# sadit/Jchemo.jl

Measured on AMD Instinct MI355X. Metric: latent-variables/sec (plskern n=1e6 p=500 q=10 nlv=25), higher is better.
Workload: dtype f64

## Files before the change

### jchemo.jl_amd/csrc/deflate.hip

```cpp
#include <stdlib.h>

#include <algorithm>

#include "jch_internal.h"

typedef double v4f64 __attribute__((ext_vector_type(4)));
#define XT_LD 65
#define YT_LD 17

template <bool APPLY, bool STORE>
__global__ __launch_bounds__(256) void k_deflate_xty(double *__restrict__ Xr, int64_t n, int p, int ldr,
                                                      const double *__restrict__ Yr, int qpad, int q, int yg0,
                                                      const double *__restrict__ d, const double *__restrict__ tcol,
                                                      const double *__restrict__ zpc, double *__restrict__ Kpart,
                                                      int kp_rows)
{
    __shared__ double xt[64 * XT_LD];
    __shared__ double yt[64 * YT_LD];
    __shared__ double tl[64], dl[64];
    const int tid = threadIdx.x, lane = tid & 63, wv = tid >> 6;
    const int j0 = blockIdx.y * 64;
    const int yg = yg0 + blockIdx.z;
    const int64_t nchunks = (n + 63) / 64;
    const int jcol = j0 + lane;
// ... 537 lines not shown
    int64_t c = blockIdx.x;
    int cur = 0;
    if (c < nchunks) { fetch(c); stage(0); }
    __syncthreads();
    for (; c < nchunks; c += gridDim.x) {
        const int64_t i0 = c * RB;
        v2f64 x[STEPS][NS];
#pragma unroll
        for (int st = 0; st < STEPS; ++st)
#pragma unroll
            for (int u = 0; u < NS; ++u) x[st][u] = xn[st][u];
        const bool more = c + gridDim.x < nchunks;
        if (more) fetch(c + gridDim.x);
#pragma unroll
        for (int st = 0; st < STEPS; ++st) {
            const int lr = 4 * st + g;
            const int64_t r = i0 + lr;
#pragma unroll
            for (int k = 0; k < MP; ++k) {
                if (k < npend) {
                    const double t = tl[cur][k][lr];
#pragma unroll
                    for (int u = 0; u < NS; ++u) {
                        x[st][u].x -= t * pk[k][u][0];
                        x[st][u].y -= t * pk[k][u][1];
                    }
                }
            }
            const double b = bt[cur][lr][c16];
#pragma unroll
            for (int u = 0; u < NS; ++u) {
                acc[u][0] = __builtin_amdgcn_mfma_f64_16x16x4f64(x[st][u].x, b, acc[u][0], 0, 0, 0);
                acc[u][1] = __builtin_amdgcn_mfma_f64_16x16x4f64(x[st][u].y, b, acc[u][1], 0, 0, 0);
            }
            if (flush && r < n) {
                double *wp = Xr + (size_t)r * (size_t)ldr;
#pragma unroll
                for (int u = 0; u < NS; ++u)
                    if (in[u]) __builtin_nontemporal_store(x[st][u], reinterpret_cast<v2f64 *>(wp + coff[u]));
            }
        }
        if (more) stage(cur ^ 1);
        __syncthreads();
        cur ^= 1;
    }
    if (Kpart) {
        double *kp = Kpart + (size_t)blockIdx.x * kp_rows * 16;
#pragma unroll
        for (int u = 0; u < NS; ++u)
#pragma unroll
            for (int h = 0; h < 2; ++h)
#pragma unroll
                for (int reg = 0; reg < 4; ++reg) {
                    const int j = 32 * (wv + 4 * u) + 2 * (4 * reg + g) + h;
                    if (j < kp_rows) kp[(size_t)j * 16 + c16] = acc[u][h][reg];
                }
    }
}

template <int NS, int STEPS, int MP>
static int32_t launch_kpass_mfma_lazy_t(jch_ctx *ctx, double *Xr, int64_t n, int p, int ldr, double *Yr, int q, const double *d,
                                        const double *pend_p, int npend, const double *tpend, int64_t tstride, const double *cvec,
                                        bool flush, double *Knext)
{
    constexpr int RB = 4 * STEPS;
    if (npend > MP) return jch_fail(ctx, JCH_EINVAL, "internal: lazy MFMA pass: %d pending corrections, at most %d", npend, MP);
    const int64_t nchunks = (n + RB - 1) / RB;
    const int nb = (int)std::max<int64_t>(std::min<int64_t>(nchunks, (int64_t)ctx->cus), 1);
    const int kp_rows = ldr;
    JCH_TRY(jch_reserve(ctx, ctx->kpart, sizeof(double) * (size_t)nb * kp_rows * 16));
    double *Kpart = (double *)ctx->kpart.ptr;
    (void)jch_ev(ctx);
    hipLaunchKernelGGL((k_kpass_mfma_lazy<NS, STEPS, MP>), dim3(nb), dim3(256), 0, ctx->stream, Xr, n, ldr, Yr, q, d, pend_p,
                       jch_nipals_lazy_pitch(ldr), npend, tpend, tstride, cvec, flush ? 1 : 0, Knext ? Kpart : nullptr, kp_rows);
    (void)jch_ev(ctx);
    if (Knext) {
        hipLaunchKernelGGL(k_reduce_kpart3, dim3((p * 16 + 63) / 64), dim3(1024), 0, ctx->stream, Kpart, nb, kp_rows * 16, p * 16, Knext);
        JCH_TRY(jch_allreduce_f64(ctx, Knext, (size_t)p * 16));
    }
    JCH_HIP(ctx, hipGetLastError());
    return JCH_OK;
}

static bool lazy_stream_shape(int ldr, int q) { return q >= 1 && q <= 4 && ldr <= 2048 && !(ldr > 1024 && q > 2); }

static int32_t launch_kpass_tile_lazy(jch_ctx *ctx, double *Xr, int64_t n, int p, int ldr, double *Yr, int qpad, int q, const double *d,
                                      const double *pend_p, int npend, const double *tpend, int64_t tstride, const double *cvec, bool flush,
                                      double *Knext)
{
    const int ptiles = (ldr + 63) / 64, kp_rows = ptiles * 64;
    const int64_t nchunks = (n + 63) / 64;
    int nbx = (ctx->cus * 3 + ptiles - 1) / ptiles;
    if (nbx > nchunks) nbx = (int)(nchunks > 0 ? nchunks : 1);
    double *Kpart = nullptr;
    if (Knext) {
        JCH_TRY(jch_reserve(ctx, ctx->kpart, sizeof(double) * (size_t)nbx * kp_rows * qpad));
        Kpart = (double *)ctx->kpart.ptr;
    }
    (void)jch_ev(ctx);
    hipLaunchKernelGGL(k_kpass_tile_lazy, dim3(nbx, ptiles, 1), dim3(256), 0, ctx->stream, Xr, n, ldr, Yr, qpad, q, d, pend_p,
                       jch_nipals_lazy_pitch(ldr), npend, tpend, tstride, cvec, flush ? 1 : 0, Kpart, kp_rows);
    (void)jch_ev(ctx);
    const int nby = (int)std::min<int64_t>((n * qpad + 255) / 256, (int64_t)ctx->cus * 8);
    hipLaunchKernelGGL(k_deflate_y, dim3(nby > 0 ? nby : 1), dim3(256), 0, ctx->stream, Yr, n, qpad, q, tpend + (size_t)(npend - 1) * tstride, cvec);
    if (Knext) {
        hipLaunchKernelGGL(k_reduce_kpart2, dim3((p * qpad + 255) / 256), dim3(256), 0, ctx->stream, Kpart, nbx, kp_rows, p, qpad, Knext);
        JCH_TRY(jch_allreduce_f64(ctx, Knext, (size_t)p * qpad));
    }
    JCH_HIP(ctx, hipGetLastError());
    return JCH_OK;
}

int32_t jch_launch_kpass_lazy(jch_ctx *ctx, double *Xr, int64_t n, int p, int ldr, double *Yr, int qpad, int q, const double *d,
                              const double *pend_p, int npend, int npend_max, const double *tpend, int64_t tstride,
                              const double *cvec, bool flush, double *Knext)
{
    if (npend < 1 || npend > npend_max || npend_max > jch_nipals_lazy_capacity(ldr, q))
        return jch_fail(ctx, JCH_EINVAL, "internal: lazy NIPALS pass: bad pending count");
    if (!lazy_stream_shape(ldr, q)) {
        if (qpad == 16 && ldr <= 1024) {
#define JCH_KM(NS, STEPS, MP) return launch_kpass_mfma_lazy_t<NS, STEPS, MP>(ctx, Xr, n, p, ldr, Yr, q, d, pend_p, npend, tpend, tstride, cvec, flush, Knext)
            if (ldr <= 128) JCH_KM(1, 4, 6);
            if (ldr <= 256) JCH_KM(2, 4, 6);
            if (ldr <= 512) JCH_KM(4, 4, 6);
            JCH_KM(8, 2, 3);
#undef JCH_KM
        }
        return launch_kpass_tile_lazy(ctx, Xr, n, p, ldr, Yr, qpad, q, d, pend_p, npend, tpend, tstride, cvec, flush, Knext);
    }
#define JCH_KL(KC, R) do { \
        if (q == 1) return launch_kpass_lazy_t<KC, R, 1>(ctx, Xr, n, p, ldr, Yr, qpad, d, pend_p, npend, npend_max, tpend, tstride, cvec, flush, Knext); \
        if (q == 2) return launch_kpass_lazy_t<KC, R, 2>(ctx, Xr, n, p, ldr, Yr, qpad, d, pend_p, npend, npend_max, tpend, tstride, cvec, flush, Knext); \
        return launch_kpass_lazy_t<KC, R, 4>(ctx, Xr, n, p, ldr, Yr, qpad, d, pend_p, npend, npend_max, tpend, tstride, cvec, flush, Knext); } while (0)
    if (ldr <= 128) JCH_KL(1, 4);
    if (ldr <= 256) JCH_KL(2, 4);
    if (ldr <= 512) JCH_KL(4, 2);
    if (ldr <= 1024) JCH_KL(8, 1);
    if (q == 1) return launch_kpass_lazy_t<16, 2, 1>(ctx, Xr, n, p, ldr, Yr, qpad, d, pend_p, npend, npend_max, tpend, tstride, cvec, flush, Knext);
    return launch_kpass_lazy_t<16, 1, 2>(ctx, Xr, n, p, ldr, Yr, qpad, d, pend_p, npend, npend_max, tpend, tstride, cvec, flush, Knext);
#undef JCH_KL
}

int32_t jch_launch_deflate(jch_ctx *ctx, double *Xr, int64_t n, int p, int ldr, double *Yr, int qpad, int q,
                           const double *d, const double *tcol, const double *zpc, double *Knext)
{
    if (q <= 4) {
#define JCH_DS(KC, R) do { \
        if (q == 1) return launch_deflate_stream<KC, R, 1>(ctx, Xr, n, p, ldr, Yr, qpad, d, tcol, zpc, Knext); \
        if (q == 2) return launch_deflate_stream<KC, R, 2>(ctx, Xr, n, p, ldr, Yr, qpad, d, tcol, zpc, Knext); \
        return launch_deflate_stream<KC, R, 4>(ctx, Xr, n, p, ldr, Yr, qpad, d, tcol, zpc, Knext); } while (0)
        if (ldr <= 128) JCH_DS(1, 4);
        if (ldr <= 256) JCH_DS(2, 4);
        if (ldr <= 512) JCH_DS(4, 2);
        if (ldr <= 1024) JCH_DS(8, 1);
        if (ldr <= 2048) {
            if (q == 1) return launch_deflate_stream<16, 2, 1>(ctx, Xr, n, p, ldr, Yr, qpad, d, tcol, zpc, Knext);
            if (q == 2) return launch_deflate_stream<16, 1, 2>(ctx, Xr, n, p, ldr, Yr, qpad, d, tcol, zpc, Knext);
        }
#undef JCH_DS
    }
    const int ptiles = (ldr + 63) / 64, kp_rows = ptiles * 64, ygroups = qpad / 16;
    const int64_t nchunks = (n + 63) / 64;
    int nbx = (ctx->cus * 3 + ptiles - 1) / ptiles;
    if (nbx > nchunks) nbx = (int)(nchunks > 0 ? nchunks : 1);
    double *Kpart = nullptr;
    if (Knext) {
        JCH_TRY(jch_reserve(ctx, ctx->kpart, sizeof(double) * (size_t)nbx * kp_rows * qpad));
        Kpart = (double *)ctx->kpart.ptr;
    }
    (void)jch_ev(ctx);
    hipLaunchKernelGGL((k_deflate_xty<true, true>), dim3(nbx, ptiles, 1), dim3(256), 0, ctx->stream, Xr, n, p, ldr, Yr, qpad,
                       q, 0, d, tcol, zpc, Kpart, kp_rows);
    (void)jch_ev(ctx);
    const int nby = (int)std::min<int64_t>((n * qpad + 255) / 256, (int64_t)ctx->cus * 8);
    hipLaunchKernelGGL(k_deflate_y, dim3(nby > 0 ? nby : 1), dim3(256), 0, ctx->stream, Yr, n, qpad, q, tcol, zpc + ldr);
    if (Knext && ygroups > 1)
        hipLaunchKernelGGL((k_deflate_xty<false, false>), dim3(nbx, ptiles, ygroups - 1), dim3(256), 0, ctx->stream, Xr, n, p,
                           ldr, Yr, qpad, q, 1, d, tcol, zpc, Kpart, kp_rows);
    if (Knext) {
        hipLaunchKernelGGL(k_reduce_kpart2, dim3((p * qpad + 255) / 256), dim3(256), 0, ctx->stream, Kpart, nbx, kp_rows, p,
                           qpad, Knext);
        JCH_TRY(jch_allreduce_f64(ctx, Knext, (size_t)p * qpad));
    }
    JCH_HIP(ctx, hipGetLastError());
    return JCH_OK;
}
```

### jchemo.jl_amd/csrc/fit.hip

```cpp
#include <stdlib.h>
#include <time.h>

#include <algorithm>
#include <condition_variable>
#include <mutex>
#include <thread>

#include "jch_internal.h"

__global__ __launch_bounds__(256) void k_fill_const(double *__restrict__ v, int m, double c)
{
    const int j = blockIdx.x * 256 + threadIdx.x;
    if (j < m) v[j] = c;
}

__global__ __launch_bounds__(256) void k_nan_zero_weight_rows(double *__restrict__ T, int64_t n, int nlv, const double *__restrict__ d)
{
    const int64_t i = (int64_t)blockIdx.x * 256 + threadIdx.x;
    if (i < n && d[i] == 0.0)
        for (int a = 0; a < nlv; ++a) T[(size_t)i + (size_t)a * (size_t)n] = __builtin_nan("");
}

__global__ __launch_bounds__(256) void k_widen_bf16(const unsigned short *__restrict__ src, int64_t ld, int64_t n, int64_t cols, double *__restrict__ dst)
{
// ... 164 lines not shown
    double tl_h2d = tl0, tl_enq = tl0, tl_sync = tl0;

    const xcopy_key xkey{io.X, (int64_t)n, (int64_t)io.ldx, p, host ? 1 : 0};
    const bool reuse_x = (d.reserved & JCH_REUSE_XCOPY) && allow_raw && ctx->xcopy_valid && ctx->xcopy == xkey && d.dtype == JCH_F64 &&
                         q + 1 <= 12 && ldr <= 512 && !jch_knob_set("JCH_NO_REUSE_XCOPY");
    if (!reuse_x) ctx->xcopy_valid = false;
    double *Xc = (double *)io.X, *Yc = (double *)io.Y;
    const double *wdev = io.weights;
    int64_t ldxc = io.ldx, ldyc = io.ldy;
    if (host) {
        JCH_TRY(jch_reserve_xstage(ctx, sizeof(double) * (size_t)n * p, reuse_x));
        JCH_TRY(jch_reserve(ctx, ctx->ystage, sizeof(double) * (size_t)n * q));
        Xc = (double *)ctx->xstage.ptr; Yc = (double *)ctx->ystage.ptr; ldxc = n; ldyc = n;
        if (!reuse_x) JCH_TRY(jch_copy2d(ctx, Xc, n, (const double *)io.X, io.ldx, n, p, hipMemcpyHostToDevice));
        JCH_TRY(jch_copy2d(ctx, Yc, n, (const double *)io.Y, io.ldy, n, q, hipMemcpyHostToDevice));
        if (io.weights) {
            JCH_TRY(jch_reserve(ctx, ctx->wstage, sizeof(double) * (size_t)n));
            JCH_HIP(ctx, hipMemcpyAsync(ctx->wstage.ptr, io.weights, sizeof(double) * (size_t)n, hipMemcpyHostToDevice, ctx->stream));
            wdev = (const double *)ctx->wstage.ptr;
        }
    }
    if (host && host_timing) { (void)hipStreamSynchronize(ctx->stream); tl_h2d = now_ms(); }
    const int nlv_cap = (int)std::min<int64_t>(d.nlv, p);
    if (d.dtype == JCH_F64) {
        JCH_TRY(jch_reserve_xr(ctx, sizeof(double) * (size_t)n * ldr, reuse_x));
        JCH_TRY(jch_reserve(ctx, ctx->yr, sizeof(double) * (size_t)n * qpad));
    }
    double *Xr = (double *)ctx->xr.ptr, *Yr = (double *)ctx->yr.ptr;
    double *dn = nullptr;
    if (!host && io.weights_norm) dn = io.weights_norm;
    else { JCH_TRY(jch_reserve(ctx, ctx->dnorm, sizeof(double) * (size_t)n)); dn = (double *)ctx->dnorm.ptr; }
    double *Tdev = nullptr;
    if (!host && io.T) Tdev = io.T;
    else { JCH_TRY(jch_reserve(ctx, ctx->tbuf, sizeof(double) * (size_t)n * nlv_cap)); Tdev = (double *)ctx->tbuf.ptr; }

    t_column_copier tcopy(ctx, (host && d.dtype == JCH_F64 && !(algo == ALGO_WOLD && (d.reserved & JCH_WOLD_REF_ZERO_WEIGHT_NAN))) ? io.T : nullptr, Tdev, n, nlv_cap);
    const size_t small_bytes = 256 * 21 + sizeof(double) * 16 * 2048 + sizeof(double) * (64 + (size_t)p + (size_t)p * qpad + 2 * (size_t)ldr + 3 * (size_t)nlv_cap * p +
                                                         (size_t)nlv_cap * q + 36 * nlv_cap + 1024 + (JCH_ZT_SLICES + 1) * ((size_t)ldr + 8 + qpad) + 2 * (size_t)(p + q) + 8 + 2 * (size_t)ldr + 128 +
                                                         (p <= JCH_SWEEP_MAXP ? jch_lv_split_doubles(p, nlv_cap) + 128 : 0));
    JCH_TRY(jch_reserve(ctx, ctx->small, small_bytes));
    jch_carve cv;
    auto take = [&](size_t count) { return (double *)ctx->small.ptr + cv.take(count); };
    jch_small s;
    s.K = take((size_t)p * qpad); s.w = take(ldr); s.r = take(ldr);
    s.P = take((size_t)nlv_cap * p); s.R = take((size_t)nlv_cap * p); s.W = take((size_t)nlv_cap * p);
    s.C = take((size_t)nlv_cap * q); s.TT = take(nlv_cap);
    s.mom = take(p + q); s.scl = take(p + q);
    double *niter_dev = take(nlv_cap);
    double *qual_dev = take(8);
    double *mshift_buf = take((size_t)ldr + 2);
    s.mshift = nullptr; s.rs = nullptr;
    const size_t out_bytes = (size_t)((char *)(qual_dev + 8) - (char *)s.P);
    double qual_host = 0.0;
    s.Z = take((size_t)nlv_cap * 16);
    const int ldz = (ldr + 1 + qpad + 7) & ~7;
    s.zt = take((size_t)JCH_ZT_SLICES * ldz); s.zpc = take((size_t)ldr + qpad);
    s.hdr = take(8);
    s.variant = 0;
    s.niter = algo == ALGO_WOLD ? niter_dev : nullptr;
    s.kr = nullptr; s.gpart = nullptr; s.lvctr = nullptr;
    auto fetch_small = [&](int k) -> int32_t {
        JCH_TRY(jch_reserve_host(ctx, out_bytes));
        char *h = (char *)ctx->hstage;
        JCH_HIP(ctx, hipMemcpyAsync(h, s.P, out_bytes, hipMemcpyDeviceToHost, ctx->stream));
        JCH_HIP(ctx, hipStreamSynchronize(ctx->stream));
        auto put = [&](double *dst, const double *dev, size_t count) {
            if (dst) memcpy(dst, h + ((const char *)dev - (const char *)s.P), sizeof(double) * count);
        };
        put(io.P, s.P, (size_t)k * p); put(io.R, s.R, (size_t)k * p);
        put(io.W, algo == ALGO_SIMP ? s.R : s.W, (size_t)k * p);
        put(io.C, s.C, (size_t)k * q); put(io.TT, s.TT, k);
        put(io.xmeans, s.mom, p); put(io.ymeans, s.mom + p, q); put(io.xscales, s.scl, p); put(io.yscales, s.scl + p, q);
        if (algo == ALGO_WOLD) put(io.niter, niter_dev, k);
        memcpy(&qual_host, h + ((const char *)qual_dev - (const char *)s.P), sizeof(double));
        return JCH_OK;
    };
    s.dbg = jch_knob_set("JCH_LV_DEBUG") ? take(512 + 16 * (nlv_cap + 2)) : nullptr;
    int defer_m = 1;
    double *pend_p = nullptr;
    if (!kern_like && d.dtype == JCH_F64) {
        defer_m = std::max(1, std::min(jch_knob("JCH_NIPALS_DEFER", JCH_NIPALS_DEFER_DEFAULT), jch_nipals_lazy_capacity(ldr, q)));
        if (defer_m > 1) pend_p = take((size_t)defer_m * jch_nipals_lazy_pitch(ldr));
    }

    const bool onepass = (d.reserved & JCH_NIPALS_ONE_PASS) != 0 && (algo == ALGO_NIPALS || algo == ALGO_WOLD);
    double *zero16 = nullptr;
    if ((d.reserved & JCH_NIPALS_ONE_PASS) && !(onepass && pend_p && !inplace))
        return jch_fail(ctx, JCH_EINVAL, "%s: JCH_NIPALS_ONE_PASS needs plsnipals / plswold with q <= 16, p <= 2048, inplace = 0, Float64", who);
    if (onepass) { zero16 = take(16); JCH_HIP(ctx, hipMemsetAsync(zero16, 0, sizeof(double) * 16, ctx->stream)); s.variant = 3; }
    if (s.dbg) JCH_HIP(ctx, hipMemsetAsync(s.dbg, 0, sizeof(double) * (512 + 16 * (nlv_cap + 2)), ctx->stream));
    if (d.dtype == JCH_BF16) {
        const bool fastb = q <= 16 && p <= JCH_SWEEP_MAXP && jch_lv_fast_lds_bytes(p, q, qpad, ldr, nlv_cap) <= 150 * 1024;
        {
            const bool fuse_b = ctx->p2p.ready && !ctx->loop;
            if (fastb && (!fuse_b || jch_lv_split_p2p_ok(ctx, p)) && jch_knob("JCH_LV_SPLIT", 1) != 0 && jch_lv_solve_lds_bytes(p, q, ldr, nlv_cap) <= 150 * 1024) {
                s.kr = take(16); JCH_TRY(jch_lv_split_begin_fit(ctx, s, take(jch_lv_split_doubles(p, nlv_cap)), p, nlv_cap));
            }
        }
        hipEvent_t evb = jch_ev(ctx);
        int nlvb = 0;
        JCH_TRY(jch_fit_plskern_bf16(ctx, d, io.X, io.ldx, io.Y, io.ldy, wdev, dn, Tdev, s, ldr, qpad, ldz, fastb, &nlvb));
        hipEvent_t eve = jch_ev(ctx);
        const size_t ev_last = ctx->ev_used - 1;
        JCH_TRY(fetch_small(nlvb));
        JCH_TRY(jch_p2p_check(ctx));
        if (io.nlv_out) *io.nlv_out = nlvb;
        if (ctx->profiling) {
            jch_profile &pr = ctx->prof;
            pr.fit_ms = ev_ms(evb, eve);
            pr.prologue_ms = ctx->ev_mark > 0 ? ev_ms(evb, ctx->ev_pool[ctx->ev_mark - 1]) : 0.0;
            double sw = 0.0; int cnt = 0;
            for (size_t i = ctx->ev_mark; i + 1 < ev_last; i += 2) { sw += ev_ms(ctx->ev_pool[i], ctx->ev_pool[i + 1]); ++cnt; }
            if (ctx->prof_stride > 1 && cnt > 0 && cnt < nlvb) { sw = sw * (double)nlvb / (double)cnt; cnt = nlvb; }
            pr.sweep_ms = sw; pr.sweep_launches = cnt; pr.nlv = nlvb;
            pr.smallstate_ms = pr.fit_ms - pr.prologue_ms - sw;
            pr.sweep_bytes = (double)n * ((p + 7) & ~7) * 2.0 + 16.0 * (double)n;
            jch_coll_collect(ctx, pr);
        }
        return JCH_OK;
    }
    hipEvent_t ev_begin = jch_ev(ctx);
    JCH_TRY(jch_launch_weights(ctx, wdev, n, dn, s.hdr, qual_dev, 8, mshift_buf, ldr + 2));
    int64_t n_total = n;
    if (ctx->nranks > 1 && n < std::min<int64_t>(p, d.nlv)) {
        double hdr_h[2];
        JCH_HIP(ctx, hipMemcpyAsync(hdr_h, s.hdr, sizeof hdr_h, hipMemcpyDeviceToHost, ctx->stream));
        JCH_HIP(ctx, hipStreamSynchronize(ctx->stream));
        n_total = (int64_t)(hdr_h[1] + 0.5);
    }
    const int nlv = (int)std::min<int64_t>(std::min<int64_t>(n_total, p), d.nlv);
    const bool fast = q <= 16 && nlv <= 1024 && p <= JCH_SWEEP_MAXP && jch_lv_fast_lds_bytes(p, q, qpad, ldr, nlv) <= 150 * 1024;
    const bool sib = algo == ALGO_SIMP || algo == ALGO_WOLD;
    const bool sib_fast = sib && jch_sibling_supported(p, q, ldr, nlv);
    const bool all_fast = sib ? (sib_fast && (algo == ALGO_SIMP || fast)) : fast;
    const int max_slices = all_fast ? JCH_ZT_SLICES : 1;
    const bool fuse_inbox = all_fast && ctx->p2p.ready && !ctx->loop &&
                            (size_t)(ldr + 1 + qpad) <= ctx->p2p.cap;
    int nslice = 1;
    const bool ext_scales = io.xscales_in != nullptr;
    const bool raw_mode = (((algo == ALGO_KERN || algo == ALGO_ROSA) && fast) || (algo == ALGO_SIMP && all_fast)) && !ext_scales && !inplace &&
                          q <= 15 && (d.reserved & ~JCH_REUSE_XCOPY) == 0 && p <= JCH_SWEEP_MAXP && allow_raw && !jch_knob_set("JCH_CENTRED_COPY");
    if (raw_mode) {
        s.mshift = mshift_buf;
        double *spread2 = take(p);
        JCH_TRY(jch_launch_pivot(ctx, Xc, ldxc, n, p, s.hdr, s.scl, spread2));
        JCH_TRY(jch_launch_moments(ctx, Yc, ldyc, nullptr, 0, dn, n, q, 0, nullptr, s.scl + p));
        bool from_copy = false;
        if (reuse_x) JCH_TRY(jch_launch_xty_rows(ctx, Xr, ldr, Yc, ldyc, dn, n, p, q, s.scl, Yr, qpad, s.K, s.mom,
                                                 s.mshift, spread2, qual_dev, s.scl, &from_copy));
        if (from_copy) ctx->xcopy_reused++;
        else {
        JCH_TRY(jch_launch_center_xty(ctx, Xc, ldxc, Yc, ldyc, dn, n, p, q, s.scl, s.mom, false, Xr, ldr, Yr, qpad, s.K, false,
                                      s.mom, s.mshift, spread2, qual_dev, s.scl));
        ctx->xcopy = xkey; ctx->xcopy_valid = true;
        }
        if (d.scal) {
            s.rs = take((size_t)ldr + 2);
            JCH_HIP(ctx, hipMemsetAsync(s.rs, 0, sizeof(double) * ((size_t)ldr + 2), ctx->stream));
            JCH_TRY(jch_launch_raw_scales(ctx, Xr, n, p, ldr, dn, s.mshift, Yr, qpad, q, s.zt, s.scl, s.K));
        }
        s.variant = 2;
    } else {
    ctx->xcopy_valid = false;
    JCH_TRY(jch_launch_moments(ctx, Xc, ldxc, Yc, ldyc, dn, n, p, q, nullptr, s.mom));
    if (ext_scales) {
        JCH_TRY(jch_reserve_host(ctx, sizeof(double) * (size_t)(p + q)));
// ... 12 lines not shown
    const size_t sweep_ev0 = ctx->ev_used;
    const bool variant2 = (d.reserved & 1) != 0;
    bool split = false;
    const bool wold_ref_nan = algo == ALGO_WOLD && (d.reserved & JCH_WOLD_REF_ZERO_WEIGHT_NAN) != 0;
    int x_reads = 0, x_writes = 0;
    if (variant2) {
        if (algo != ALGO_KERN || !fast) return jch_fail(ctx, JCH_EINVAL, "%s: variant 2 needs plskern with q <= 16 and p <= %d", who, JCH_SWEEP_MAXP);
        JCH_TRY(jch_reserve(ctx, ctx->gram, sizeof(double) * (size_t)p * ldr));
        double *G = (double *)ctx->gram.ptr;
        JCH_TRY(jch_launch_syrk(ctx, Xr, n, p, ldr, dn, G, ldr));
        s.variant = 1;
        JCH_TRY(jch_launch_lv_update(ctx, s, p, q, qpad, ldr, -1, nlv, 0, 1, ldz, true));
        for (int a = 0; a < nlv; ++a) {
            JCH_TRY(jch_launch_gmatvec(ctx, G, ldr, p, ldr, s.r, s.zt));
            JCH_TRY(jch_launch_lv_update(ctx, s, p, q, qpad, ldr, a, nlv, 0, 1, ldz, true));
        }
        JCH_TRY(jch_launch_scores(ctx, Xr, n, p, ldr, s.R, nlv, Tdev));
    } else {
    if (algo == ALGO_SIMP && all_fast) JCH_TRY(jch_launch_lv_update_simp(ctx, s, p, q, ldr, -1, nlv, 1, ldz));
    else if (algo == ALGO_SIMP) JCH_TRY(jch_launch_lv_update(ctx, s, p, q, qpad, ldr, -1, nlv, 2, 1, ldz, false));
    else if (algo == ALGO_WOLD && all_fast) JCH_TRY(jch_launch_wold_b(ctx, s, p, q, ldr, 0, nlv, io.tol, io.maxit));
    else if (algo == ALGO_WOLD) JCH_TRY(jch_launch_lv_update(ctx, s, p, q, qpad, ldr, 0 | 0x20000000, nlv, 4, 1, ldz, false, false, nullptr, 0, 0, io.tol, io.maxit));
    else {
        split = (algo == ALGO_KERN || algo == ALGO_ROSA) && fast && jch_knob("JCH_LV_SPLIT", 1) != 0 &&
                jch_lv_solve_lds_bytes(p, q, ldr, nlv) <= 150 * 1024 && (!fuse_inbox || jch_lv_split_p2p_ok(ctx, p));
        if (split) { s.kr = take(16); JCH_TRY(jch_lv_split_begin_fit(ctx, s, take(jch_lv_split_doubles(p, nlv)), p, nlv)); }
        JCH_TRY(jch_launch_lv_update(ctx, s, p, q, qpad, ldr, -1, nlv, kern_like ? 0 : 1, 1, ldz, fast));
    }
    int npend = 0, pend_a0 = 0;
    if (pend_p) JCH_HIP(ctx, hipMemsetAsync(pend_p, 0, sizeof(double) * (size_t)defer_m * jch_nipals_lazy_pitch(ldr), ctx->stream));
    for (int a = 0; a < nlv; ++a) {
        double *tcol = Tdev + (size_t)a * (size_t)n;
        if (kern_like) {
            jch_part_view pv;
            const bool split_fused = split && fuse_inbox;
            JCH_TRY(jch_launch_sweep(ctx, Xr, n, p, ldr, dn, s.rs ? s.rs : s.r, Yr, qpad, 0, tcol, s.zt, ldz, max_slices, &nslice, raw_mode ? s.mshift : nullptr,
                                     split && (ctx->nranks == 1 || split_fused) ? &pv : nullptr));
            tcopy.column_done(a);
            if (ctx->nranks > 1 && max_slices > 1) nslice = JCH_ZT_SLICES;
            if (split) {
                if (!pv.part) {
                    if (!split_fused) JCH_TRY(jch_allreduce_slices(ctx, s.zt, ldr + 1 + (raw_mode ? 1 : 0), nslice, ldz, &nslice));
                    pv.part = s.zt; pv.nb = nslice; pv.ldpart = ldz;
                }
                if (split_fused) ctx->coll_transport = JCH_TRANSPORT_INBOX_FUSED;
                JCH_TRY(jch_launch_lv_split(ctx, s, p, q, ldr, a, nlv, pv.part, pv.nb, pv.ldpart, ldr, raw_mode ? ldr + 1 : -1, raw_mode ? 1 : 0, a + 1 < nlv, split_fused));
                continue;
            }
            if (fuse_inbox && algo != ALGO_SIMP) {
                ctx->coll_transport = JCH_TRANSPORT_INBOX_FUSED;
                JCH_TRY(jch_launch_lv_update(ctx, s, p, q, qpad, ldr, a, nlv, 0, nslice, ldz, fast, true));
            } else {
                JCH_TRY(jch_allreduce_slices(ctx, s.zt, ldr + 1 + (raw_mode ? 1 : 0), nslice, ldz, &nslice));
                if (algo == ALGO_SIMP && all_fast) JCH_TRY(jch_launch_lv_update_simp(ctx, s, p, q, ldr, a, nlv, nslice, ldz));
                else if (algo == ALGO_SIMP) JCH_TRY(jch_launch_lv_update(ctx, s, p, q, qpad, ldr, a, nlv, 2, nslice, ldz, false));
                else JCH_TRY(jch_launch_lv_update(ctx, s, p, q, qpad, ldr, a, nlv, 0, nslice, ldz, fast));
            }
        } else {
            if (pend_p) JCH_TRY(jch_launch_sweep_lazy(ctx, Xr, n, ldr, dn, s.w, Yr, qpad, tcol, s.zt, ldz, max_slices, &nslice, pend_p, npend,
                                                      defer_m - 1, Tdev + (size_t)pend_a0 * (size_t)n, n));
            else if (qpad > 64) {
                JCH_TRY(jch_launch_sweep(ctx, Xr, n, p, ldr, dn, s.w, Yr, qpad, 0, tcol, s.zt, ldz, max_slices, &nslice));
                JCH_TRY(jch_launch_ytdt(ctx, Yr, n, qpad, dn, tcol, s.zt + ldr + 1));
            } else JCH_TRY(jch_launch_sweep(ctx, Xr, n, p, ldr, dn, s.w, Yr, qpad, q, tcol, s.zt, ldz, max_slices, &nslice));
            tcopy.column_done(a);
            if (ctx->nranks > 1 && max_slices > 1) nslice = JCH_ZT_SLICES;
            ++x_reads;
            if (fuse_inbox) {
                ctx->coll_transport = JCH_TRANSPORT_INBOX_FUSED;
                JCH_TRY(jch_launch_lv_update(ctx, s, p, q, qpad, ldr, a | 0x40000000, nlv, 1, nslice, ldz, fast, true));
            } else {
                JCH_TRY(jch_allreduce_slices(ctx, s.zt, ldr + 1 + qpad, nslice, ldz, &nslice));
                JCH_TRY(jch_launch_lv_update(ctx, s, p, q, qpad, ldr, a | 0x40000000, nlv, 1, nslice, ldz, fast));
            }
            const bool last = a + 1 == nlv;
            if (!last || inplace) {
                if (pend_p && onepass) {
                    if (npend == 0) pend_a0 = a;
                    JCH_HIP(ctx, hipMemcpyAsync(pend_p + (size_t)npend * jch_nipals_lazy_pitch(ldr), s.zpc, sizeof(double) * (size_t)ldr,
                                                hipMemcpyDeviceToDevice, ctx->stream));
                    ++npend;
                    if (npend == defer_m && !last) {
                        JCH_TRY(jch_launch_kpass_lazy(ctx, Xr, n, p, ldr, Yr, qpad, q, dn, pend_p, npend, defer_m,
                                                      Tdev + (size_t)pend_a0 * (size_t)n, n, zero16, true, nullptr));
                        npend = 0; ++x_writes; ++x_reads;
                    }
                    --x_reads;
                } else
                if (pend_p) {
                    if (npend == 0) pend_a0 = a;
                    JCH_HIP(ctx, hipMemcpyAsync(pend_p + (size_t)npend * jch_nipals_lazy_pitch(ldr), s.zpc, sizeof(double) * (size_t)ldr,
                                                hipMemcpyDeviceToDevice, ctx->stream));
                    ++npend;
                    const bool flush = npend == defer_m || last;
                    JCH_TRY(jch_launch_kpass_lazy(ctx, Xr, n, p, ldr, Yr, qpad, q, dn, pend_p, npend, defer_m,
                                                  Tdev + (size_t)pend_a0 * (size_t)n, n, s.zpc + ldr, flush, last ? nullptr : s.K));
                    if (flush) { npend = 0; ++x_writes; }
                } else {
                    JCH_TRY(jch_launch_deflate(ctx, Xr, n, p, ldr, Yr, qpad, q, dn, tcol, s.zpc, last ? nullptr : s.K));
                    ++x_writes;
                }
                ++x_reads;
            }
            if (!last) {
                if (algo == ALGO_WOLD && all_fast) JCH_TRY(jch_launch_wold_b(ctx, s, p, q, ldr, a + 1, nlv, io.tol, io.maxit));
                else if (algo == ALGO_WOLD) JCH_TRY(jch_launch_lv_update(ctx, s, p, q, qpad, ldr, (a + 1) | 0x20000000, nlv, 4, 1, ldz, false, false, nullptr, 0, 0, io.tol, io.maxit));
                else JCH_TRY(jch_launch_lv_update(ctx, s, p, q, qpad, ldr, (a + 1) | 0x20000000, nlv, 1, 1, ldz, fast));
            }
        }
    }
    }
    if (wold_ref_nan) {
        hipLaunchKernelGGL(k_nan_zero_weight_rows, dim3((unsigned)((n + 255) / 256)), dim3(256), 0, ctx->stream, Tdev, n, nlv, dn);
        JCH_HIP(ctx, hipGetLastError());
    }
    if (algo == ALGO_ROSA) JCH_TRY(jch_launch_rosa_orthw(ctx, s.W, p, nlv));
    if (algo == ALGO_NIPALS || algo == ALGO_WOLD || algo == ALGO_ROSA) JCH_TRY(jch_launch_nipals_R(ctx, s, p, nlv));
    hipEvent_t ev_end = jch_ev(ctx);
    const size_t sweep_ev1 = ctx->ev_used;

    if (!kern_like && inplace) {
        JCH_TRY(jch_launch_export_colmajor(ctx, Xr, ldr, Yr, qpad, n, p, q, Xc, ldxc, Yc, ldyc, algo == ALGO_WOLD ? dn : nullptr));
    }
    if (algo == ALGO_ROSA && inplace) JCH_TRY(jch_launch_ydeflate_all(ctx, Yc, ldyc, Tdev, n, s.C, q, nlv));
    auto d2h = [&](double *dst, const double *src, size_t count) -> int32_t {
        if (dst) JCH_HIP(ctx, hipMemcpyAsync(dst, src, sizeof(double) * count, hipMemcpyDeviceToHost, ctx->stream));
        return JCH_OK;
    };
    if (host) {
        if (!tcopy.active() || variant2) JCH_TRY(d2h(io.T, Tdev, (size_t)n * nlv));
        JCH_TRY(d2h(io.weights_norm, dn, (size_t)n));
        if (inplace) {
            JCH_TRY(jch_copy2d(ctx, (double *)io.X, io.ldx, Xc, n, n, p, hipMemcpyDeviceToHost));
            JCH_TRY(jch_copy2d(ctx, (double *)io.Y, io.ldy, Yc, n, n, q, hipMemcpyDeviceToHost));
        }
    }
    tl_enq = now_ms();
    JCH_TRY(fetch_small(nlv));
    tl_sync = now_ms();
    if (tcopy.active() && !tcopy.finish(!variant2, nlv)) return jch_fail(ctx, JCH_EHIP, "%s: copying the scores to the host failed", who);
    JCH_TRY(jch_p2p_check(ctx));
    if (raw_mode && !(qual_host <= JCH_PIVOT_MAX_RATIO)) {
        ctx->pivot_refits++;
        return fit_impl(ctx, io, algo, false);
    }
    if (io.nlv_out) *io.nlv_out = nlv;
    if (host && host_timing)
        fprintf(stderr, "[jch] host-arrays fit: H2D %.1f ms | enqueue %.1f ms | device drain + small outputs %.1f ms | score columns still in flight %.1f ms | total %.1f ms\n",
                tl_h2d - tl0, tl_enq - tl_h2d, tl_sync - tl_enq, now_ms() - tl_sync, now_ms() - tl0);
    if (s.dbg) {
        std::vector<double> h(nlv + 1);
        (void)hipMemcpy(h.data(), s.dbg, sizeof(double) * (nlv + 1), hipMemcpyDeviceToHost);
        fprintf(stderr, "[jch] jacobi sweeps per LV:");
        for (int i = 0; i < nlv; ++i) fprintf(stderr, " %d", (int)h[i]);
        fprintf(stderr, "\n");
        std::vector<double> st(16 * (nlv + 1));
        (void)hipMemcpy(st.data(), s.dbg + 512, sizeof(double) * st.size(), hipMemcpyDeviceToHost);
        for (int c : {0, 1, nlv / 2, nlv - 1}) {
            fprintf(stderr, "[jch] lv_update call %d stamps (cycles since kernel start):", c);
            for (int k = 1; k < 16; ++k) if (st[16 * c + k] > 0) fprintf(stderr, " %d:%.0f", k, st[16 * c + k] - st[16 * c]);
            fprintf(stderr, "\n");
        }
    }

    if (ctx->profiling) {
        jch_profile &pr = ctx->prof;
        pr.fit_ms = ev_ms(ev_begin, ev_end);
        pr.prologue_ms = ev_ms(ev_begin, ev_prologue);
        pr.nlv = nlv;
        double sw = 0.0; int cnt = 0;
        for (size_t i = sweep_ev0; i + 1 < sweep_ev1; i += 2) { sw += ev_ms(ctx->ev_pool[i], ctx->ev_pool[i + 1]); ++cnt; }
        const bool sampled = kern_like && !variant2 && ctx->prof_stride > 1;
        if (sampled) sw = cnt > 0 ? sw * (double)nlv / (double)cnt : 0.0;
        pr.sweep_ms = sw;
        pr.sweep_launches = variant2 ? 1 : (kern_like ? (sampled ? (cnt > 0 ? nlv : 0) : cnt) : nlv);
        pr.smallstate_ms = pr.fit_ms - pr.prologue_ms - sw;
        const double per_x = (double)n * ldr * 8.0;
        pr.sweep_bytes = kern_like ? per_x + 16.0 * (double)n : per_x * (double)(x_reads + x_writes) / (double)std::max(nlv, 1);
        jch_coll_collect(ctx, pr);
// ... 104 lines not shown
```

### jchemo.jl_amd/csrc/jch_internal.h

```cpp
#pragma once
#include <hip/hip_runtime.h>
#include <stdint.h>
#include <stdio.h>
#include <string.h>

#include <functional>
#include <string>
#include <vector>

#include "jchemo_hip.h"

#define JCH_MAXQ 64
#define JCH_ZT_SLICES 8
#define JCH_SWEEP_MAXP 2048

struct xcopy_key {
    const void *X; int64_t n, ldx; int p, host;
    bool operator==(const xcopy_key &o) const { return X == o.X && n == o.n && ldx == o.ldx && p == o.p && host == o.host; }
};
struct jch_buf {
    void *ptr = nullptr;
    size_t bytes = 0;
};

// ... 128 lines not shown
}
int32_t jch_reserve_host(jch_ctx *ctx, size_t bytes);
int32_t jch_allreduce_f64(jch_ctx *ctx, double *dev_buf, size_t count);
struct jch_comm_off {
    jch_ctx *ctx;
    void *comm, *loop;
    int nranks, rank;
    bool p2p_ready;
    explicit jch_comm_off(jch_ctx *c) : ctx(c), comm(c->comm), loop(c->loop), nranks(c->nranks), rank(c->rank), p2p_ready(c->p2p.ready)
    {
        c->comm = nullptr; c->loop = nullptr; c->nranks = 1; c->rank = 0; c->p2p.ready = false;
    }
    ~jch_comm_off()
    {
        ctx->comm = comm; ctx->loop = loop; ctx->nranks = nranks; ctx->rank = rank;
        ctx->p2p.ready = p2p_ready && !(ctx->p2p.host_status && *ctx->p2p.host_status != 0ull);
    }
    jch_comm_off(const jch_comm_off &) = delete;
    jch_comm_off &operator=(const jch_comm_off &) = delete;
};
int32_t jch_allreduce_slices(jch_ctx *ctx, double *zt, int m, int nslice, int ldz, int *nslice_out);
int32_t jch_p2p_allreduce(jch_ctx *ctx, const double *src, size_t count, int nslice, int ldz, double *dst);
int32_t jch_p2p_check(jch_ctx *ctx);
void jch_p2p_destroy(jch_ctx *ctx);

struct jch_span {
    hipEvent_t a = nullptr, b = nullptr;
};
hipEvent_t jch_ev(jch_ctx *ctx);
bool jch_prof_sample(jch_ctx *ctx);
void jch_coll_begin(jch_ctx *ctx);
void jch_coll_end(jch_ctx *ctx);
void jch_coll_reset(jch_ctx *ctx);
void jch_coll_collect(jch_ctx *ctx, jch_profile &pr);

struct jch_part_view {
    const double *part = nullptr;
    int nb = 0, ldpart = 0;
};

int32_t jch_launch_weights(jch_ctx *ctx, const double *w_dev , int64_t n, double *dnorm,
                           double *hdr , double *zero0 = nullptr, int nzero0 = 0,
                           double *zero1 = nullptr, int nzero1 = 0 );
int32_t jch_launch_moments(jch_ctx *ctx, const double *Xc, int64_t ldx, const double *Yc, int64_t ldy,
                           const double *d, int64_t n, int p, int q, const double *means ,
                           double *out , bool do_sqrt = true);
int32_t jch_launch_center_xty(jch_ctx *ctx, double *Xc, int64_t ldx, double *Yc, int64_t ldy, const double *d,
                              int64_t n, int p, int q, const double *mom, const double *scl, bool writeback,
                              double *Xr, int ldr, double *Yr, int qpad, double *K , bool scal,
                              double *means_out = nullptr ,
                              double *mshift_out = nullptr ,
                              const double *spread2 = nullptr ,
                              double *qual = nullptr ,
                              double *ones_out = nullptr );
int32_t jch_launch_pivot(jch_ctx *ctx, const double *Xc, int64_t ldx, int64_t n, int p, const double *hdr ,
                         double *pivot , double *spread2 );
int32_t jch_launch_export_colmajor(jch_ctx *ctx, const double *Xr, int ldr, const double *Yr, int qpad, int64_t n,
                                   int p, int q, double *Xc, int64_t ldx, double *Yc, int64_t ldy,
                                   const double *sqrt_rowscale = nullptr );
int32_t jch_launch_sweep(jch_ctx *ctx, const double *Xr, int64_t n, int p, int ldr, const double *d, const double *rvec,
                         const double *Yr, int qpad, int q_extra ,
                         double *tcol, double *zt , int ldz, int max_slices,
                         int *nslice_out, const double *mu = nullptr ,
                         jch_part_view *pv = nullptr );
int32_t jch_launch_reduce_rows(jch_ctx *ctx, const double *part, int nb, int ldpart, int m, double *out);
int32_t jch_launch_xty_rows(jch_ctx *ctx, const double *Xr, int ldr, const double *Yc, int64_t ldy, const double *d, int64_t n, int p, int q,
                            const double *mom, double *Yr, int qpad, double *K, double *means_out, double *mshift_out,
                            const double *spread2, double *qual, double *ones_out, bool *done);
int32_t jch_launch_raw_scales(jch_ctx *ctx, const double *Xr, int64_t n, int p, int ldr, const double *d, const double *mshift,
                              const double *Yr, int qpad, int q, double *tmp, double *scl, double *K);
int32_t jch_launch_reduce_part8(jch_ctx *ctx, const double *part, int nb, int ldpart, int m, double *zt, int ldz, int *nslice_out);
int32_t jch_launch_sweep_wide(jch_ctx *ctx, const double *Xr, int64_t n, int ldr, const double *d, const double *rvec,
                              const double *Yr, int qpad, bool nipals, double *tcol, double *zt);
int32_t jch_launch_ytdt(jch_ctx *ctx, const double *Yr, int64_t n, int qpad, const double *d, const double *tcol, double *out );
#define JCH_NIPALS_DEFER_DEFAULT 6
static inline int jch_nipals_lazy_pitch(int ldr) { return 128 * (ldr <= 128 ? 1 : ldr <= 256 ? 2 : ldr <= 512 ? 4 : ldr <= 1024 ? 8 : 16); }
int32_t jch_sweep_tickets(jch_ctx *ctx, int **out);
int jch_nipals_lazy_capacity(int ldr, int q);
int32_t jch_launch_sweep_lazy(jch_ctx *ctx, const double *Xr, int64_t n, int ldr, const double *d, const double *wvec,
                              const double *Yr, int qpad, double *tcol, double *zt, int ldz, int max_slices, int *nslice_out,
                              const double *pend_p, int npend, int npend_max, const double *tpend, int64_t tstride);
int32_t jch_launch_kpass_lazy(jch_ctx *ctx, double *Xr, int64_t n, int p, int ldr, double *Yr, int qpad, int q, const double *d,
                              const double *pend_p, int npend, int npend_max, const double *tpend, int64_t tstride,
                              const double *cvec, bool flush, double *Knext);
int32_t jch_launch_deflate(jch_ctx *ctx, double *Xr, int64_t n, int p, int ldr, double *Yr, int qpad, int q,
                           const double *d, const double *tcol, const double *zpc ,
                           double *Knext );
struct jch_small {
    double *K;
    double *w, *r;
    double *P, *R, *W;
    double *C;
    double *TT;
    double *Z;
    double *zt;
    double *zpc;
    double *mom, *scl;
    double *mshift;
    double *rs;
    double *hdr;
    int variant;
    double *dbg;
    double *niter;
    double *kr;
    double *gpart;
    unsigned *lvctr;
};

int32_t jch_launch_lv_update(jch_ctx *ctx, const jch_small &s, int p, int q, int qpad, int ldr, int a ,
                             int nlv, int algo , int nslice, int ldz, bool fast, bool fuse_p2p = false,
                             const double *bf_src = nullptr, int bf_ld = 0, int bf_ldr = 0, double tol = 0.0, int maxit = 0);
size_t jch_lv_fast_lds_bytes(int p, int q, int qpad, int ldr, int nlv);
int32_t jch_launch_lv_update_fast(jch_ctx *ctx, const jch_small &s, int p, int q, int qpad, int ldr, int a, int nlv, int algo,
                                  int do_a, int do_b, int nslice, int ldz, bool fuse_p2p = false, const double *bf_src = nullptr,
                                  int bf_ld = 0, int bf_ldr = 0);
int jch_lv_split_blocks(int p);
int jch_lv_split_gld(int nlv);
size_t jch_lv_split_doubles(int p, int nlv);
int32_t jch_lv_split_begin_fit(jch_ctx *ctx, jch_small &s, double *gbuf, int p, int nlv);
size_t jch_lv_solve_lds_bytes(int p, int q, int ldr, int nlv);
int32_t jch_launch_lv_split(jch_ctx *ctx, const jch_small &s, int p, int q, int ldr, int a, int nlv, const double *part, int nb,
                            int ldpart, int itt, int ist , int mode , bool solve,
                            bool fuse_p2p = false );
bool jch_lv_split_p2p_ok(const jch_ctx *ctx, int p);
struct p2p_dev;
void jch_p2p_next(jch_ctx *ctx, p2p_dev *out);
int32_t jch_launch_nipals_R(jch_ctx *ctx, const jch_small &s, int p, int nlv);
bool jch_sibling_supported(int p, int q, int ldr, int nlv);
int32_t jch_launch_lv_update_simp(jch_ctx *ctx, const jch_small &s, int p, int q, int ldr, int a , int nlv, int nslice, int ldz);
int32_t jch_launch_wold_b(jch_ctx *ctx, const jch_small &s, int p, int q, int ldr, int a, int nlv, double tol, int maxit);
int32_t jch_launch_rosa_orthw(jch_ctx *ctx, double *W, int p, int nlv);
int32_t jch_launch_ydeflate_all(jch_ctx *ctx, double *Yc, int64_t ldy, const double *T, int64_t n, const double *C, int q, int nlv);
int32_t jch_launch_affine_gemm(jch_ctx *ctx, const double *Xc, int64_t m, int p, int64_t ldx, const double *Bs ,
                               int k, int kpad, const double *bias , double *out, int64_t ldo);
int32_t jch_launch_weighted_ss(jch_ctx *ctx, const double *Xc, int64_t n, int p, int64_t ldx, const double *d,
                               const double *shift, const double *iscale, double *out1);
int32_t jch_fit_plskern_bf16(jch_ctx *ctx, const jch_pls_desc &d, const void *Xv, int64_t ldx, const void *Yv, int64_t ldy,
                             const double *wdev, double *dn, double *Tdev, jch_small &s, int ldr_small, int qpad, int ldz,
                             bool fast, int *nlv_out);
int32_t jch_launch_syrk(jch_ctx *ctx, const double *Xr, int64_t n, int p, int ldr, const double *d, double *G, int ldg);
int32_t jch_launch_gmatvec(jch_ctx *ctx, const double *G, int ldg, int p, int ldr, const double *r, double *out);
int32_t jch_launch_scores(jch_ctx *ctx, const double *Xr, int64_t n, int p, int ldr, const double *Rm, int nlv, double *T);
int32_t jch_launch_kgram(jch_ctx *ctx, int kind, const double *Z, int64_t m, int64_t ldz, const double *zdiv, const double *X, int64_t n,
                         int64_t ldx, const double *xdiv, int64_t p, double gamma, double coef0, int degree, bool sym, double *K, int64_t ldk);
int32_t jch_launch_kgram_prep(jch_ctx *ctx, const double *X, int64_t n, int64_t ldx, int64_t p, const double *c, double *cp, int64_t ldc, int64_t pp, double *nrm);
int32_t jch_launch_kp_centred_gram(jch_ctx *ctx, int kind, double gamma, double coef0, int degree, const double *X, int64_t n, int64_t ldx,
                                   const double *xdiv, int64_t p, const double *wn, double *Kraw, double *Kc, double *vt, double *sdev);
int32_t jch_launch_kc_panel(jch_ctx *ctx, const double *Kc, int64_t n, int64_t ldk, const double *V, int64_t ldv, int b, const double *d,
                            double *out, int64_t ldo);
struct jch_eig_lead_out {
    int b = 0, niter = 0;
    bool converged = false;
    std::vector<double> theta, resid;
    double *X = nullptr;
    double *AX = nullptr;
    const double *theta_dev = nullptr;
    double *scratch = nullptr;
};
int32_t jch_eig_lead(jch_ctx *ctx, const double *A, int64_t dim, int64_t lda, const double *sqrtw, int nlv, double tol, int maxit, jch_eig_lead_out *out);
int32_t jch_launch_xtdx(jch_ctx *ctx, const double *X, int64_t n, int p, int64_t ldx, const double *mu, const double *d, double *G, int64_t ldg);
int32_t jch_colselect_reserve(jch_ctx *ctx, int64_t p);
int32_t jch_launch_col_median_mad(jch_ctx *ctx, const double *X, int64_t n, int64_t p, int64_t ldx, double *med, double *mad);
int32_t jch_launch_weiszfeld_dist(jch_ctx *ctx, const double *X, int64_t n, int p, int64_t ldx, const double *c, const double *sdiv, double *d);
int32_t jch_spatial_median_dev(jch_ctx *ctx, const double *X, int64_t n, int p, int64_t ldx, double delta, int maxit, double *mu_dev, double *d_dev, int32_t *niter,
                               double *h_last, int32_t *converged);
int32_t jch_check_kernel(jch_ctx *ctx, const char *who, int32_t kind, int32_t degree);
int32_t jch_launch_divcols(jch_ctx *ctx, double *A, int64_t lda, int64_t n, int64_t cols, const double *s_dev);
// ... 56 lines not shown
```

Baseline: 1543.

## Add register-pipelined streaming K-pass kernel for q 5-12 lazy NIPALS

Adds a new streaming kernel for the deferred-deflation K pass. Each wave multi-buffers rows of X in registers, applies the pending rank-one corrections from LDS, updates Y, and accumulates X'DY per column in registers instead of using the MFMA tile path. The default knob routes it only for ldr 257-512 and q 9-10, which is the benchmark shape (p=500, q=10). It adds a per-block partial reduction through LDS and a separate reduce kernel, and its heavy register use could hurt occupancy.

```diff
diff --git a/jchemo.jl_amd/csrc/deflate.hip b/jchemo.jl_amd/csrc/deflate.hip
--- a/jchemo.jl_amd/csrc/deflate.hip
+++ b/jchemo.jl_amd/csrc/deflate.hip
@@ -643,7 +643,202 @@
     return JCH_OK;
 }
 
+__device__ __forceinline__ v2f64 jch_kp_take(const v2f64 &a)
+{
+    typedef int jch_v4i __attribute__((ext_vector_type(4)));
+    const jch_v4i in = __builtin_bit_cast(jch_v4i, a);
+    int o0, o1, o2, o3;
+    asm("v_accvgpr_read_b32 %0, %1" : "=v"(o0) : "a"(in.x));
+    asm("v_accvgpr_read_b32 %0, %1" : "=v"(o1) : "a"(in.y));
+    asm("v_accvgpr_read_b32 %0, %1" : "=v"(o2) : "a"(in.z));
+    asm("v_accvgpr_read_b32 %0, %1" : "=v"(o3) : "a"(in.w));
+    return __builtin_bit_cast(v2f64, jch_v4i{o0, o1, o2, o3});
+}
+template <int KC, int R, int NBUF, int Q, int RP>
+__global__ __launch_bounds__(256) void k_kpass_stream(double *__restrict__ Xr, int64_t n, int ldr, double *__restrict__ Yr, int q,
+                                                      const double *__restrict__ dw, const double *__restrict__ pend_p, int npend,
+                                                      const double *__restrict__ tpend, int64_t tstride, const double *__restrict__ cvec,
+                                                      int flush, double *__restrict__ part, int ldpart)
+{
+    extern __shared__ __attribute__((aligned(16))) double red[];
+    constexpr int LDP = KC * 128, YL = (R + 3) / 4, QH = Q / 2;
+    static_assert(R % 4 == 0 && R % RP == 0 && Q % 2 == 0 && Q <= 16, "k_kpass_stream: groups of 4 rows, an even Q of at most one Y row");
+    const int lane = threadIdx.x & 63, wv = __builtin_amdgcn_readfirstlane(threadIdx.x >> 6);
+    const int lrow = lane >> 4, ly = lane & 15;
+    v2f64 kacc[Q][KC];
+    int coff[KC];
+#pragma unroll
+    for (int k = 0; k < KC; ++k) {
+        const int col = 2 * lane + 128 * k;
+        coff[k] = col < ldr ? col : ldr - 2;
+#pragma unroll
+        for (int y = 0; y < Q; ++y) kacc[y][k] = v2f64{0.0, 0.0};
+    }
+    const int64_t ngroups = (n + R - 1) / R;
+    const int64_t gstride = (int64_t)gridDim.x * 4;
+    const int knew = npend - 1;
+    const int pl = min(lane, npend * R - 1);
+    const int64_t pk_off = (int64_t)(pl / R) * tstride;
+    const int pr = pl % R;
+    v2f64 X[NBUF][R][KC];
+    double Yb[NBUF][YL], Db[NBUF][YL], Tb[NBUF];
+    double cf = 0.0;
+    auto fetch = [&](v2f64 (&xb)[R][KC], double (&yb)[YL], double (&db)[YL], double &tb, int64_t gg) {
+        const int64_t r0 = (gg < ngroups ? gg : ngroups - 1) * R;
+#pragma unroll
+        for (int j = 0; j < YL; ++j) {
+            const int64_t row = r0 + lrow + 4 * j < n ? r0 + lrow + 4 * j : n - 1;
+            yb[j] = Yr[(size_t)row * 16 + ly];
+            db[j] = dw[row];
+        }
+        tb = tpend[pk_off + (r0 + pr < n ? r0 + pr : n - 1)];
+#pragma unroll
+        for (int rr = 0; rr < R; ++rr) {
+            const int64_t row = r0 + rr < n ? r0 + rr : n - 1;
+            const double *rp = Xr + (size_t)row * (size_t)ldr;
+#pragma unroll
+            for (int k = 0; k < KC; ++k) xb[rr][k] = __builtin_nontemporal_load(reinterpret_cast<const v2f64 *>(rp + coff[k]));
+        }
+    };
+    auto process = [&](v2f64 (&xb)[R][KC], double (&yb)[YL], double (&db)[YL], double tpc, int64_t gg) {
+        const int64_t row0 = gg * R;
+        double yv[YL];
+#pragma unroll
+        for (int j = 0; j < YL; ++j) {
+            double tl = 0.0;
+#pragma unroll
+            for (int rr = 4 * j; rr < 4 * j + 4; ++rr) tl = lrow == (rr & 3) ? jch_kp_readlane(tpc, knew * R + rr) : tl;
+            const int64_t row = row0 + lrow + 4 * j;
+            const double yn = yb[j] - tl * cf;
+            const bool live = row < n;
+            if (live && ly < q) Yr[(size_t)row * 16 + ly] = yn;
+            yv[j] = live ? db[j] * yn : 0.0;
+        }
+#pragma unroll
+        for (int h = 0; h < R; h += RP) {
+            v2f64 x[RP][KC];
+#pragma unroll
+            for (int rr = 0; rr < RP; ++rr)
+#pragma unroll
+                for (int kk = 0; kk < KC; ++kk) x[rr][kk] = jch_kp_take(xb[h + rr][kk]);
+            for (int k = 0; k < npend; ++k) {
+                double tk[RP];
+#pragma unroll
+                for (int rr = 0; rr < RP; ++rr) tk[rr] = jch_kp_readlane(tpc, k * R + h + rr);
+                const double *pl_k = red + k * LDP + 2 * lane;
+#pragma unroll
+                for (int kk = 0; kk < KC; ++kk) {
+                    const v2f64 pf = *reinterpret_cast<const v2f64 *>(pl_k + 128 * kk);
+#pragma unroll
+                    for (int rr = 0; rr < RP; ++rr) {
+                        x[rr][kk].x -= tk[rr] * pf.x;
+                        x[rr][kk].y -= tk[rr] * pf.y;
+                    }
+                }
+            }
+#pragma unroll
+            for (int r2 = 0; r2 < RP; ++r2) {
+                const int rr = h + r2;
+                const int64_t row = row0 + rr;
+                if (row < n) {
+                    if (flush) {
+                        double *wp = Xr + (size_t)row * (size_t)ldr;
+#pragma unroll
+                        for (int k = 0; k < KC; ++k)
+                            if (2 * lane + 128 * k < ldr) __builtin_nontemporal_store(x[r2][k], reinterpret_cast<v2f64 *>(wp + 2 * lane + 128 * k));
+                    }
+#pragma unroll
+                    for (int y = 0; y < Q; ++y) {
+                        const double s = jch_kp_readlane(yv[rr >> 2], 16 * (rr & 3) + y);
+#pragma unroll
+                        for (int k = 0; k < KC; ++k) {
+                            kacc[y][k].x += s * x[r2][k].x;
+                            kacc[y][k].y += s * x[r2][k].y;
+                        }
+                    }
+                }
+            }
+        }
+    };
+    constexpr int NB1 = NBUF - 1;
+    int64_t g = (int64_t)blockIdx.x * 4 + wv;
+#pragma unroll
+    for (int b = 0; b < NB1; ++b) fetch(X[b], Yb[b], Db[b], Tb[b], g + b * gstride);
+    for (int e = threadIdx.x; e < npend * LDP; e += 256) red[e] = pend_p[e];
+    cf = ly < q ? cvec[ly] : 0.0;
+    __syncthreads();
+    for (; g < ngroups; g += NBUF * gstride) {
+#pragma unroll
+        for (int b = 0; b < NBUF; ++b) {
+            fetch(X[(b + NB1) % NBUF], Yb[(b + NB1) % NBUF], Db[(b + NB1) % NBUF], Tb[(b + NB1) % NBUF], g + (b + NB1) * gstride);
+            process(X[b], Yb[b], Db[b], Tb[b], g + b * gstride);
+        }
+    }
+    if (!part) return;
+    double *prow = part + (size_t)blockIdx.x * ldpart;
+#pragma unroll
+    for (int h = 0; h < 2; ++h) {
+        __syncthreads();
+#pragma unroll
+        for (int y = 0; y < QH; ++y) {
+#pragma unroll
+            for (int k = 0; k < KC; ++k)
+                *reinterpret_cast<v2f64 *>(red + (size_t)(wv * QH + y) * LDP + 2 * lane + 128 * k) = kacc[h * QH + y][k];
+        }
+        __syncthreads();
+        const int ny = min(QH, q - h * QH);
+        for (int e = threadIdx.x; e < ny * ldr; e += 256) {
+            const int y = e / ldr, c = e - y * ldr;
+            double s = 0.0;
+#pragma unroll
+            for (int w = 0; w < 4; ++w) s += red[(size_t)(w * QH + y) * LDP + c];
+            prow[(size_t)(h * QH + y) * ldr + c] = s;
+        }
+    }
+}
+
+template <int KC, int R, int NBUF, int Q, int RP>
+static int32_t launch_kpass_stream_t(jch_ctx *ctx, double *Xr, int64_t n, int p, int ldr, double *Yr, int q, const double *d,
+                                     const double *pend_p, int npend, int npend_max, const double *tpend, int64_t tstride,
+                                     const double *cvec, bool flush, double *Knext)
+{
+    static_assert(6 * R <= 64, "the scores of 6 pending corrections x R rows live in one wave's lanes");
+    const size_t lds_red = sizeof(double) * 4 * (Q / 2) * KC * 128;
+    const size_t lds = std::max(lds_red, sizeof(double) * (size_t)npend_max * KC * 128);
+    static int bpc = 0;
+    static jch_per_device_once once;
+    if (!once.done(ctx->device)) {
+        JCH_HIP(ctx, hipFuncSetAttribute((const void *)k_kpass_stream<KC, R, NBUF, Q, RP>, hipFuncAttributeMaxDynamicSharedMemorySize, 160 * 1024));
+        int nblk = 0;
+        hipError_t e = hipOccupancyMaxActiveBlocksPerMultiprocessor(&nblk, k_kpass_stream<KC, R, NBUF, Q, RP>, 256, lds_red);
+        bpc = (e == hipSuccess && nblk > 0) ? nblk : 1;
+        once.mark(ctx->device);
+    }
+    if (npend_max * R > 64 || lds > 160 * 1024) return jch_fail(ctx, JCH_EINVAL, "internal: streaming NIPALS pass: %d pending corrections, %zu bytes of LDS", npend_max, lds);
+    const int use_bpc = std::max(1, std::min<int>(bpc, (int)((160 * 1024) / lds)));
+    const int64_t ngroups = (n + R - 1) / R;
+    const int nb = (int)std::max<int64_t>(std::min<int64_t>((ngroups + 3) / 4, (int64_t)ctx->cus * use_bpc), 1);
+    const int ldpart = (q * ldr + 7) & ~7;
+    double *part = nullptr;
+    if (Knext) {
+        JCH_TRY(jch_reserve(ctx, ctx->kpart, sizeof(double) * (size_t)nb * ldpart));
+        part = (double *)ctx->kpart.ptr;
+    }
+    (void)jch_ev(ctx);
+    hipLaunchKernelGGL((k_kpass_stream<KC, R, NBUF, Q, RP>), dim3(nb), dim3(256), lds, ctx->stream, Xr, n, ldr, Yr, q, d, pend_p, npend, tpend,
+                       tstride, cvec, flush ? 1 : 0, part, ldpart);
+    (void)jch_ev(ctx);
+    if (Knext) {
+        hipLaunchKernelGGL(k_reduce_kstream, dim3((q * ldr + 63) / 64), dim3(1024), 0, ctx->stream, part, nb, ldpart, ldr, p, q, 16, Knext);
+        JCH_TRY(jch_allreduce_f64(ctx, Knext, (size_t)p * 16));
+    }
+    JCH_HIP(ctx, hipGetLastError());
+    return JCH_OK;
+}
+
 static bool lazy_stream_shape(int ldr, int q) { return q >= 1 && q <= 4 && ldr <= 2048 && !(ldr > 1024 && q > 2); }
+static bool kpass_stream_envelope(int ldr, int qpad, int q) { return qpad == 16 && q > 4 && q <= 12 && ldr <= 512; }
+static bool kpass_stream_adopted(int ldr, int q) { return ldr > 256 && ldr <= 512 && q >= 9 && q <= 10; }
 
 static int32_t launch_kpass_tile_lazy(jch_ctx *ctx, double *Xr, int64_t n, int p, int ldr, double *Yr, int qpad, int q, const double *d,
                                       const double *pend_p, int npend, const double *tpend, int64_t tstride, const double *cvec, bool flush,
@@ -674,11 +869,20 @@
 
 int32_t jch_launch_kpass_lazy(jch_ctx *ctx, double *Xr, int64_t n, int p, int ldr, double *Yr, int qpad, int q, const double *d,
                               const double *pend_p, int npend, int npend_max, const double *tpend, int64_t tstride,
-                              const double *cvec, bool flush, double *Knext)
+                              const double *cvec, bool flush, double *Knext, int kstream)
 {
     if (npend < 1 || npend > npend_max || npend_max > jch_nipals_lazy_capacity(ldr, q))
         return jch_fail(ctx, JCH_EINVAL, "internal: lazy NIPALS pass: bad pending count");
     if (!lazy_stream_shape(ldr, q)) {
+        if (kstream != 0 && kpass_stream_envelope(ldr, qpad, q) && (kstream == 1 || kpass_stream_adopted(ldr, q))) {
+#define JCH_KS(KC, R, NB, Q, RP) return launch_kpass_stream_t<KC, R, NB, Q, RP>(ctx, Xr, n, p, ldr, Yr, q, d, pend_p, npend, npend_max, tpend, tstride, cvec, flush, Knext)
+#define JCH_KSQ(KC, R, NB, RP12) do { if (q <= 8) JCH_KS(KC, R, NB, 8, 4); if (q <= 10) JCH_KS(KC, R, NB, 10, 4); JCH_KS(KC, R, NB, 12, RP12); } while (0)
+            if (ldr <= 128) JCH_KSQ(1, 8, 2, 4);
+            if (ldr <= 256) JCH_KSQ(2, 8, 3, 4);
+            JCH_KSQ(4, 4, 3, 2);
+#undef JCH_KSQ
+#undef JCH_KS
+        }
         if (qpad == 16 && ldr <= 1024) {
 #define JCH_KM(NS, STEPS, MP) return launch_kpass_mfma_lazy_t<NS, STEPS, MP>(ctx, Xr, n, p, ldr, Yr, q, d, pend_p, npend, tpend, tstride, cvec, flush, Knext)
             if (ldr <= 128) JCH_KM(1, 4, 6);
diff --git a/jchemo.jl_amd/csrc/fit.hip b/jchemo.jl_amd/csrc/fit.hip
--- a/jchemo.jl_amd/csrc/fit.hip
+++ b/jchemo.jl_amd/csrc/fit.hip
@@ -270,6 +270,7 @@
         defer_m = std::max(1, std::min(jch_knob("JCH_NIPALS_DEFER", JCH_NIPALS_DEFER_DEFAULT), jch_nipals_lazy_capacity(ldr, q)));
         if (defer_m > 1) pend_p = take((size_t)defer_m * jch_nipals_lazy_pitch(ldr));
     }
+    const int kstream = jch_knob("JCH_KPASS_STREAM", -1);
 
     const bool onepass = (d.reserved & JCH_NIPALS_ONE_PASS) != 0 && (algo == ALGO_NIPALS || algo == ALGO_WOLD);
     double *zero16 = nullptr;
@@ -448,7 +449,7 @@
                     ++npend;
                     if (npend == defer_m && !last) {
                         JCH_TRY(jch_launch_kpass_lazy(ctx, Xr, n, p, ldr, Yr, qpad, q, dn, pend_p, npend, defer_m,
-                                                      Tdev + (size_t)pend_a0 * (size_t)n, n, zero16, true, nullptr));
+                                                      Tdev + (size_t)pend_a0 * (size_t)n, n, zero16, true, nullptr, kstream));
                         npend = 0; ++x_writes; ++x_reads;
                     }
                     --x_reads;
@@ -460,7 +461,7 @@
                     ++npend;
                     const bool flush = npend == defer_m || last;
                     JCH_TRY(jch_launch_kpass_lazy(ctx, Xr, n, p, ldr, Yr, qpad, q, dn, pend_p, npend, defer_m,
-                                                  Tdev + (size_t)pend_a0 * (size_t)n, n, s.zpc + ldr, flush, last ? nullptr : s.K));
+                                                  Tdev + (size_t)pend_a0 * (size_t)n, n, s.zpc + ldr, flush, last ? nullptr : s.K, kstream));
                     if (flush) { npend = 0; ++x_writes; }
                 } else {
                     JCH_TRY(jch_launch_deflate(ctx, Xr, n, p, ldr, Yr, qpad, q, dn, tcol, s.zpc, last ? nullptr : s.K));
diff --git a/jchemo.jl_amd/csrc/jch_internal.h b/jchemo.jl_amd/csrc/jch_internal.h
--- a/jchemo.jl_amd/csrc/jch_internal.h
+++ b/jchemo.jl_amd/csrc/jch_internal.h
@@ -234,7 +234,7 @@
                               const double *pend_p, int npend, int npend_max, const double *tpend, int64_t tstride);
 int32_t jch_launch_kpass_lazy(jch_ctx *ctx, double *Xr, int64_t n, int p, int ldr, double *Yr, int qpad, int q, const double *d,
                               const double *pend_p, int npend, int npend_max, const double *tpend, int64_t tstride,
-                              const double *cvec, bool flush, double *Knext);
+                              const double *cvec, bool flush, double *Knext, int kstream);
 int32_t jch_launch_deflate(jch_ctx *ctx, double *Xr, int64_t n, int p, int ldr, double *Yr, int qpad, int q,
                            const double *d, const double *tcol, const double *zpc ,
                            double *Knext );
```

New measurement: 1545 (median of 6 runs). About the same (+0.1%).
